# quentinll/pertrenderer

Hardware: AMD Instinct MI355X
Metric: rendered frames/sec + ms/backward, 256² img, 50 faces/px, 8 samples (higher is better)
Workload: dtype f32; 1 GPU; cfg2 pose-opt step: sphere_642 (1280 faces), 256x256, faces_per_pixel=50, Sr=Sa=8 Gaussian, sigma=1e-3 gamma=1e-2, blur=ln(1e4-1)*sigma, fwd + L2 loss (native) + bwd + Adam step on the pose (lr 5e-2); image_size=256, faces_per_pixel=50, nb_samples=8, rast_samples=8, batch=1, execution=graph, parallelism=single GPU

## Files before the change

### pertrenderer_amd/csrc/pr_rast.hip

```cpp
#include <cstdlib>
#include <type_traits>

#include <hip/hip_fp16.h>

#include "pr_common.h"

namespace pr {
namespace {

constexpr float kEps = 1e-8f;
constexpr int kTile = 4;

struct V2 {
  float x, y;
};

template <bool FAST = false>
PR_DEV float dv(float a, float b) {
  if constexpr (FAST) return a * __builtin_amdgcn_rcpf(b);
  else return a / b;
}

PR_DEV float edge_fn(V2 p, V2 a, V2 b) { return (p.x - a.x) * (b.y - a.y) - (p.y - a.y) * (b.x - a.x); }

// ... 396 lines not shown
        const int je = j >> 6;
#pragma unroll
        for (int e = 0; e < E; ++e) {
          const int pe = e ^ je;
          if (pe > e) {
            const bool up = ((e * 64 + lane) & k) == 0;
            const float a = key[e], b = key[pe];
            if ((a > b) == up) {
              key[e] = b; key[pe] = a;
              const int t = val[e]; val[e] = val[pe]; val[pe] = t;
            }
          }
        }
      } else {
#pragma unroll
        for (int e = 0; e < E; ++e) {
          const float ok = __shfl_xor(key[e], j);
          const int ov = __shfl_xor(val[e], j);
          const int i = e * 64 + lane;
          const bool up = (i & k) == 0, lower = (lane & j) == 0;
          const bool take = lower == up ? (ok < key[e]) : (ok > key[e]);
          if (take) { key[e] = ok; val[e] = ov; }
        }
      }
    }
  }
}

template <int E>
PR_DEV void wave_sort_lds(float* lkey, int* lidx, int lane) {
  float kk[E];
  int vv[E];
#pragma unroll
  for (int e = 0; e < E; ++e) { kk[e] = lkey[e * 64 + lane]; vv[e] = lidx[e * 64 + lane]; }
  wave_bitonic_sort<E>(kk, vv, lane);
#pragma unroll
  for (int e = 0; e < E; ++e) { lkey[e * 64 + lane] = kk[e]; lidx[e * 64 + lane] = vv[e]; }
}

PR_DEV bool ekey_less(float2 x, float2 y) { return key_less(x.x, __float_as_int(x.y), y.x, __float_as_int(y.y)); }

template <int SL>
PR_HD size_t rast_fwd_wave_bytes(int K) {
  using C = RastCfg<SL>;
  const size_t b = C::CH * sizeof(FaceRec) + (size_t)K * (64 / SL + rast_qpad<SL>()) * 8 + 64 * 4 + C::CH * 12;
  return (b + 15) / 16 * 16;
}

template <int SL>
size_t rast_fwd_lds_sl(int K, int NW) {
  return NW * rast_fwd_wave_bytes<SL>(K) + (size_t)RastCfg<SL>::CAP * 12 + 16;
}

size_t rast_fwd_lds(int K, int SL, int NW = 1) {
  return SL == 8 ? rast_fwd_lds_sl<8>(K, 1)
                 : SL == 4 ? rast_fwd_lds_sl<4>(K, NW) : (SL == 2 ? rast_fwd_lds_sl<2>(K, 1) : rast_fwd_lds_sl<1>(K, 1));
}

template <int SL>
PR_DEV int from_slice(int v, int s) {
  if constexpr (SL == 1) {
    return v;
  } else if constexpr (SL == 2) {
    switch (s) {
      case 0: return __builtin_amdgcn_update_dpp(0, v, 0xA0, 0xf, 0xf, false);
      default: return __builtin_amdgcn_update_dpp(0, v, 0xF5, 0xf, 0xf, false);
    }
  } else if constexpr (SL == 8) {
    return __shfl(v, (int)(__lane_id() & ~7u) | s);
  } else {
    switch (s) {
      case 0: return __builtin_amdgcn_update_dpp(0, v, 0x00, 0xf, 0xf, false);
      case 1: return __builtin_amdgcn_update_dpp(0, v, 0x55, 0xf, 0xf, false);
      case 2: return __builtin_amdgcn_update_dpp(0, v, 0xAA, 0xf, 0xf, false);
      default: return __builtin_amdgcn_update_dpp(0, v, 0xFF, 0xf, 0xf, false);
    }
  }
}

template <int SL>
PR_DEV int quad_rot(int v, int r) {
  if constexpr (SL == 2) {
    return __builtin_amdgcn_update_dpp(0, v, 0xB1, 0xf, 0xf, false);
  } else if constexpr (SL == 8) {
    const unsigned l = __lane_id();
    return __shfl(v, (int)((l & ~7u) | ((l + (unsigned)r) & 7u)));
  } else {
    switch (r) {
      case 1: return __builtin_amdgcn_update_dpp(0, v, 0x39, 0xf, 0xf, false);
      case 2: return __builtin_amdgcn_update_dpp(0, v, 0x4E, 0xf, 0xf, false);
      default: return __builtin_amdgcn_update_dpp(0, v, 0x93, 0xf, 0xf, false);
    }
  }
}

PR_DEV int64_t uniform64(int64_t v) {
  return (int64_t)(((uint64_t)(uint32_t)__builtin_amdgcn_readfirstlane((int)(v >> 32)) << 32) |
                   (uint32_t)__builtin_amdgcn_readfirstlane((int)v));
}

PR_DEV void ring_tile(int b, int m, int& tx, int& ty) {
  int r = (int)(__builtin_sqrtf((float)b) * 0.5f);
  while (4 * (r + 1) * (r + 1) <= b) ++r;
  while (4 * r * r > b) --r;
  const int k = b - 4 * r * r, s = 2 * r + 2, c0 = m / 2 - r - 1;
  if (k < s) { tx = c0 + k; ty = c0; }
  else if (k < 2 * s - 2) { tx = c0 + s - 1; ty = c0 + 1 + (k - s); }
  else if (k < 3 * s - 2) { tx = c0 + s - 1 - (k - (2 * s - 2)); ty = c0 + s - 1; }
  else { tx = c0; ty = c0 + s - 2 - (k - (3 * s - 2)); }
}

#ifndef PR_RAST_WPE
#define PR_RAST_WPE 1
#endif
#ifndef PR_RAST_DUO_WPE
#define PR_RAST_DUO_WPE 1
#endif
template <int SL, bool PERSP, bool CLIP, bool FRAG, int NW>
__global__ void __launch_bounds__(64 * NW, NW == 2 ? PR_RAST_DUO_WPE : PR_RAST_WPE)
    rast_fwd_kernel(PRRastArgs a, const FaceRec* __restrict__ faces, const uint2* __restrict__ fbox,
                    int chunk_cull, int ring, BinGrid bins) {
  constexpr int TW = SL >= 4 ? 4 : 8, TH = 64 / SL / TW, TP = TW * TH;
  constexpr int kCap = RastCfg<SL>::CAP, kGroup = RastCfg<SL>::G, CH = RastCfg<SL>::CH;
  constexpr int QS = TP + rast_qpad<SL>();
  constexpr int NT = 64 * NW;
  extern __shared__ float smem[];
  const int K = a.K;
  const int tid = threadIdx.x, lane = tid & 63, wv = NW == 2 ? tid >> 6 : 0;
  const int pix = lane / SL, slice = lane % SL;
  const size_t wbytes = rast_fwd_wave_bytes<SL>(K);
  char* wbase = reinterpret_cast<char*>(smem) + wv * wbytes;
  FaceRec* lrec = reinterpret_cast<FaceRec*>(wbase);
  float2* q = reinterpret_cast<float2*>(lrec + CH);
  int* qsz = reinterpret_cast<int*>(q + (size_t)K * QS);
  int* lcf = qsz + 64;
  float* lcs = reinterpret_cast<float*>(lcf + CH);
  float* lmg = lcs + CH;
  int* lfid = reinterpret_cast<int*>(reinterpret_cast<char*>(smem) + NW * wbytes);
  float* lkey = reinterpret_cast<float*>(lfid + kCap);
  float* lsuf = lkey;
  int* lidx = reinterpret_cast<int*>(lkey + kCap);
  int64_t* lctl = reinterpret_cast<int64_t*>(lidx + kCap);
  int* lscr = reinterpret_cast<int*>(lctl);
  const int n = blockIdx.z;
  const int H = a.H, W = a.W;
  int tile_x = blockIdx.x, tile_y = blockIdx.y;
  if (ring & 1) {
    const int b = blockIdx.y * gridDim.x + blockIdx.x;
    if (gridDim.y == gridDim.x) {
      ring_tile(b, gridDim.x, tile_x, tile_y);
    } else {
      ring_tile(b >> 1, gridDim.x, tile_x, tile_y);
      tile_y = 2 * tile_y + (b & 1);
    }
  }
  const int row0 = tile_y * TH, col0 = tile_x * TW;
  const int row = row0 + pix / TW, col = col0 + pix % TW;
  const bool inimg = row < H && col < W;
  const V2 p{ndc(W - 1 - min(col, W - 1), W, H), ndc(H - 1 - min(row, H - 1), H, W)};
  const int c1 = min(col0 + TW - 1, W - 1), r1 = min(row0 + TH - 1, H - 1);
  const float txmax = ndc(W - 1 - col0, W, H), txmin = ndc(W - 1 - c1, W, H);
  const float tymax = ndc(H - 1 - row0, H, W), tymin = ndc(H - 1 - r1, H, W);
  const float tcx = 0.5f * (txmin + txmax), tcy = 0.5f * (tymin + tymax);
  const float ptile = fmaxf(fmaxf(fabsf(txmin), fabsf(txmax)), fmaxf(fabsf(tymin), fabsf(tymax)));
  const int64_t fb = a.mesh_first_face[n];
  const int* ids = nullptr;
  int64_t fe = a.mesh_num_faces[n];
  if (bins.count) {
    const int b = (n * bins.ny + row0 / bins.bs) * bins.nx + col0 / bins.bs;
    const int c = bins.count[b];
    if (c <= bins.cap) { ids = bins.list + (int64_t)b * bins.cap; fe = c; }
  }
  constexpr bool clip = CLIP;
  const float blur = a.blur_radius_dev ? *a.blur_radius_dev : a.blur_radius, sqrt_blur = sqrtf(blur);
  int qs = 0;
  float qlast_z = __builtin_inff();
  int qlast_f = 0x7fffffff;
  int64_t base = 0;
#ifdef PR_RAST_PROFILE
  long long stamp[6] = {0, 0, 0, 0, 0, 0}, t_ = __builtin_amdgcn_s_memtime();
  const long long rt0 = __builtin_amdgcn_s_memrealtime();
  int nlist = 0, n_app = 0, n_ins = 0, w_ins = 0;
#endif
  while (base < fe) {
    int nl = 0;
    if (__builtin_amdgcn_readfirstlane(ids == nullptr && wv == 0)) {
      const int64_t ufb = uniform64(fb), ufe = uniform64(fe);
      const int f_lo = (int)ufb, f_hi = (int)(ufb + ufe);
      const int cN = (int)((ufb + ufe - 1) / kChunk) + 1;
      int64_t ub = uniform64(base);
      int un = 0;
      while (ub < ufe && un <= kCap - 64) {
        const int c0 = (int)((ufb + ub) / kChunk);
        bool ck = c0 + lane < cN;
        if (ck && chunk_cull) {
          const float4 cb = unpack_box(fbox[(c0 + lane) * kChunk]);
          ck = !(cb.x > txmax || cb.y < txmin || cb.z > tymax || cb.w < tymin);
        }
        uint64_t live = __ballot(ck);
        const int64_t wend = (int64_t)(c0 + 64 < cN ? c0 + 64 : cN) * kChunk - ufb;
        int64_t next = wend;
        while (live != 0 && un <= kCap - 64) {
          uint2 pb[kChunkU];
          const uint64_t live0 = live;
          const int nlive = __popcll(live);
          const int np = nlive < kChunkU ? nlive : kChunkU;
          int g = -1;
#pragma unroll
          for (int u = 0; u < kChunkU; ++u) {
            pb[u] = make_uint2(0u, 0u);
            if (u < np) {
              const int f0 = (c0 + __builtin_ctzll(live)) * kChunk, f = f0 + lane;
              live &= live - 1;
              pb[u] = fbox[f >= f_lo && f < f_hi ? f : f_lo];
              if (lane == u) g = f0;
            }
          }
          float4 ex = make_float4(0.f, 0.f, 0.f, 0.f);
          if (g >= f_lo && g < f_hi) ex = exact_box(faces + g);
          uint64_t lv = live0;
          int stop = -1;
#pragma unroll
          for (int u = 0; u < kChunkU; ++u) {
            if (u < np && stop < 0) {
              const uint64_t lv0 = lv;
              const int f = (c0 + __builtin_ctzll(lv)) * kChunk + lane;
              lv &= lv - 1;
              float4 bb = unpack_box(pb[u]);
              const float e0 = __shfl(ex.x, u), e1 = __shfl(ex.y, u), e2 = __shfl(ex.z, u), e3 = __shfl(ex.w, u);
              if (lane == 0) bb = make_float4(e0, e1, e2, e3);
              const bool keep = f >= f_lo && f < f_hi && !(bb.x > txmax || bb.y < txmin || bb.z > tymax || bb.w < tymin);
              const uint64_t bal = __ballot(keep);
              const int cnt = __popcll(bal);
              if (un + cnt > kCap) {
                stop = u;
                live = lv0;
              } else {
                *(keep ? lfid + un + __popcll(bal & ((1ull << lane) - 1ull)) : lscr) = f;
                un += cnt;
              }
            }
          }
          next = live != 0 ? (int64_t)(c0 + __builtin_ctzll(live)) * kChunk - ufb : wend;
          if (stop >= 0) live = 0;
        }
        next = next > ub ? next : ub;
        ub = next < ufe ? next : ufe;
      }
      base = ub;
      nl = un;
    }
    while (wv == 0 && base < fe && nl <= kCap - 64) {
      uint2 pb[kCullU];
      int fi[kCullU];
#pragma unroll
      for (int u = 0; u < kCullU; ++u) {
        const int64_t i = base + u * 64 + lane;
        const int64_t ic = i < fe ? i : fe - 1;
        fi[u] = ids ? ids[ic] : (int)(fb + ic);
      }
#pragma unroll
      for (int u = 0; u < kCullU; ++u) pb[u] = fbox[fi[u]];
      int64_t next = base + 64 * kCullU;
      bool stop = false;
#pragma unroll
      for (int u = 0; u < kCullU; ++u) {
        const int64_t i = base + u * 64 + lane;
        float4 bb = unpack_box(pb[u]);
        if ((fi[u] & (kChunk - 1)) == 0) bb = exact_box(faces + fi[u]);
        const bool keep = i < fe && !(bb.x > txmax || bb.y < txmin || bb.z > tymax || bb.w < tymin);
        const uint64_t bal = __ballot(keep);
        const int cnt = __popcll(bal);
        if (!stop && nl + cnt > kCap) { stop = true; next = base + u * 64; }
        if (!stop) {
          if (keep) lfid[nl + __popcll(bal & ((1ull << lane) - 1ull))] = fi[u];
          nl += cnt;
        }
      }
      base = next < fe ? next : fe;
    }
    if constexpr (NW > 1) {
      if (tid == 0) { lctl[0] = base; lctl[1] = nl; }
      __syncthreads();
      base = lctl[0];
      nl = (int)lctl[1];
    }
    __syncthreads();
    PR_STAMP(0);
#ifdef PR_RAST_PROFILE
    nlist += nl;
#endif
    if (nl == 0) continue;
    if (ring & 2) {
      const int t = ring >> 8;
      if (nl >= t + 32) __builtin_amdgcn_s_setprio(3);
      else if (nl >= t + 16) __builtin_amdgcn_s_setprio(2);
      else if (nl >= t) __builtin_amdgcn_s_setprio(1);
    }
    bool done = !inimg;
    int n2 = 64;
    while (n2 < nl) n2 <<= 1;
    for (int i = tid; i < n2; i += NT) {
      float key = __builtin_inff();
      if (i < nl) {
        const FaceRec& r = faces[lfid[i]];
        const float4 ra = r.a, rb = r.b, re = r.e, rf = r.f;
        const float z2 = r.c.x, area = r.d.y;
        const float e0 = (tcx - ra.w) * re.w - (tcy - rb.x) * re.z;
        const float e1 = (tcx - rb.z) * rf.y - (tcy - rb.w) * rf.x;
        const float e2 = (tcx - ra.x) * re.y - (tcy - ra.y) * re.x;
        const float ia = 1.f / area;
        const float zc = (e0 * ia) * ra.z + (e1 * ia) * rb.y + (e2 * ia) * z2;
        const float zmx = fmaxf(ra.z, fmaxf(rb.y, z2));
        key = fminf(fmaxf(zc, rf.w), zmx);
        if (key != key) key = rf.w;
        key = fminf(key, 3.0e38f);
        if (key != key) key = 0.f;
      }
      lkey[i] = key;
      lidx[i] = i < nl ? i : 0x7fffffff;
    }
    __syncthreads();
    PR_STAMP(1);
    if (wv == 0) {
      if (n2 == 64) wave_sort_lds<1>(lkey, lidx, lane);
      else if (kCap >= 128 && n2 == 128) wave_sort_lds<2>(lkey, lidx, lane);
      else if (kCap >= 256 && n2 == 256) wave_sort_lds<4>(lkey, lidx, lane);
      else if constexpr (kCap >= 512) wave_sort_lds<8>(lkey, lidx, lane);
    }
    __syncthreads();
    PR_STAMP(2);
    {
      const int per = (nl + 63) / 64;
      const int i0 = lane * per, i1 = wv == 0 ? min(nl, i0 + per) : i0;
      float zl[8];
#pragma unroll
      for (int u = 0; u < 8; ++u) zl[u] = i0 + u < i1 ? faces[lfid[lidx[i0 + u]]].f.w : __builtin_inff();
      float m = __builtin_inff();
#pragma unroll
      for (int u = 0; u < 8; ++u) m = fminf(m, zl[u]);
      float ex = m;
#pragma unroll
      for (int o = 1; o < 64; o <<= 1) {
        const float t = __shfl_down(ex, o);
        if (lane + o < 64) ex = fminf(ex, t);
      }
      float run = __shfl_down(ex, 1);
      if (lane == 63) run = __builtin_inff();
      __syncthreads();
#pragma unroll
      for (int u = 7; u >= 0; --u) {
        run = fminf(run, zl[u]);
        if (i0 + u < i1) lsuf[i0 + u] = run;
      }
    }
    __syncthreads();
    PR_STAMP(3);
    float4 nra, nrb, nrc, nrd, nre, nrf;
    int nfid = 0;
    float nsuf = 0.f;
    if (lane < CH) {
      const int sp = min(wv * CH + lane, nl - 1);
      nfid = lfid[lidx[sp]];
      nsuf = lsuf[sp];
      const FaceRec* fp = faces + nfid;
      nra = fp->a; nrb = fp->b; nrc = fp->c; nrd = fp->d; nre = fp->e; nrf = fp->f;
    }
    for (int c0 = wv * CH; c0 < nl && __ballot(!done) != 0; c0 += NW * CH) {
      const int cnt = min(CH, nl - c0);
      __builtin_amdgcn_wave_barrier();
      if (lane < cnt) {
        FaceRec& d = lrec[lane];
        d.a = nra; d.b = nrb; d.c = nrc; d.d = nrd; d.e = nre; d.f = nrf;
        lcf[lane] = nfid;
        lcs[lane] = nsuf;
        if constexpr (!PERSP) lmg[lane] = dist_margin(nra, nrb, ptile, sqrt_blur, blur);
      }
      __builtin_amdgcn_fence(__ATOMIC_RELEASE, "wavefront");
      __builtin_amdgcn_wave_barrier();
      if (c0 + NW * CH < nl && lane < CH) {
        const int sp = c0 + NW * CH + min(lane, nl - c0 - NW * CH - 1);
        nfid = lfid[lidx[sp]];
        nsuf = lsuf[sp];
        const FaceRec* fp = faces + nfid;
        nra = fp->a; nrb = fp->b; nrc = fp->c; nrd = fp->d; nre = fp->e; nrf = fp->f;
      }
      const int steps = (cnt + SL - 1) / SL;
      for (int t = 0; t < steps; t += kGroup) {
        bool cand[kGroup], ok[kGroup];
        float pzv[kGroup];
        int idx[kGroup];
        FaceRec rr[kGroup];
        bool any = false;
#pragma unroll
        for (int j = 0; j < kGroup; ++j) {
          idx[j] = (t + j) * SL + slice;
          ok[j] = idx[j] < cnt;
          rr[j] = lrec[min(idx[j], cnt - 1)];
        }
        bool maybe[kGroup];
        float dfast[kGroup], mg[kGroup];
#pragma unroll
        for (int j = 0; j < kGroup; ++j) {
          dfast[j] = 0.f;
          mg[j] = PERSP ? 0.f : lmg[min(idx[j], cnt - 1)];
          if constexpr (PERSP) maybe[j] = ok[j] && in_bbox(rr[j], p);
          else maybe[j] = ok[j] && face_maybe(rr[j], p, blur, mg[j], dfast[j]);
          any |= __ballot(maybe[j]) != 0;
        }
// ... 108 lines not shown
            const bool enter = mine && !done && cand[j] && (qs < K || key_less(pz, fid, qlast_z, qlast_f));
            if (__ballot(enter) == 0) continue;
            {
              if (enter) {
                if (qs == 0 || key_less(qlast_z, qlast_f, pz, fid)) {
                  q[qs * QS + pix] = make_float2(pz, __int_as_float(fid));
                  ++qs;
                  qlast_z = pz;
                  qlast_f = fid;
#ifdef PR_RAST_PROFILE
                  ++n_app;
#endif
                } else {
#ifdef PR_RAST_PROFILE
                  ++n_ins;
#endif
                  int pos = qs < K ? qs : K - 1;
                  if (qs < K) ++qs;
                  while (pos > 0) {
                    float2 e[4];
#pragma unroll
                    for (int i = 0; i < 4; ++i) e[i] = q[max(pos - 1 - i, 0) * QS + pix];
                    int sh = 0;
#pragma unroll
                    for (int i = 0; i < 4; ++i) {
                      if (sh == i && pos - 1 - i >= 0 && key_less(pz, fid, e[i].x, __float_as_int(e[i].y))) {
                        q[(pos - i) * QS + pix] = e[i];
                        sh = i + 1;
                      }
                    }
                    pos -= sh;
                    if (sh < 4) break;
                  }
                  q[pos * QS + pix] = make_float2(pz, __int_as_float(fid));
                  const float2 last = q[(qs - 1) * QS + pix];
                  qlast_z = last.x;
                  qlast_f = __float_as_int(last.y);
                }
              }
            }
            if constexpr (SL > 1) {
              qs = from_slice<SL>(qs, sl);
              qlast_z = __int_as_float(from_slice<SL>(__float_as_int(qlast_z), sl));
              qlast_f = from_slice<SL>(qlast_f, sl);
            }
          }
        }
#ifdef PR_RAST_PROFILE
        w_ins += __ballot(n_ins != ins_before) != 0;
#endif
        if (__ballot(!done) == 0) break;
      }
    }
    __syncthreads();
    PR_STAMP(4);
  }
  if (slice == 0) qsz[pix] = inimg ? qs : 0;
  if constexpr (NW == 1) {
    if (slice == 0 && inimg && a.pix_count) a.pix_count[((int64_t)n * H + row) * W + col] = qs;
  }
  __syncthreads();
  const float2* qa = reinterpret_cast<const float2*>(reinterpret_cast<const char*>(lrec) - wv * wbytes + CH * sizeof(FaceRec));
  const float2* qb = reinterpret_cast<const float2*>(reinterpret_cast<const char*>(qa) + wbytes);
  const int* qsa = reinterpret_cast<const int*>(qa + (size_t)K * QS);
  const int* qsb = reinterpret_cast<const int*>(qb + (size_t)K * QS);
  if constexpr (NW == 2) {
    if (wv == 0 && slice == 0 && inimg && a.pix_count)
      a.pix_count[((int64_t)n * H + row) * W + col] = min(K, qsa[pix] + qsb[pix]);
  }
  auto msize = [&](int t) { return NW == 2 ? min(K, qsa[t] + qsb[t]) : qsz[t]; };
  auto kth = [&](int t, int k) -> float2 {
    if constexpr (NW == 1) {
      return q[k * QS + t];
    } else {
      const int na = qsa[t], nb = qsb[t];
      int lo = max(0, k - nb), hi = min(k, na);
      while (lo < hi) {
        const int mid = (lo + hi) >> 1;
        if (ekey_less(qa[mid * QS + t], qb[(k - 1 - mid) * QS + t])) lo = mid + 1;
        else hi = mid;
      }
      const int j = k - lo;
      if (lo >= na) return qb[j * QS + t];
      if (j >= nb) return qa[lo * QS + t];
      const float2 x = qa[lo * QS + t], y = qb[j * QS + t];
      return ekey_less(x, y) ? x : y;
    }
  };
  {
    const int ncols = min(TW, W - col0), nrows = min(TH, H - row0);
    const int per_row = ncols * K, total = nrows * per_row;
    const float inv_row = 1.f / (float)per_row, inv_k = 1.f / (float)K;
#ifndef PR_RAST_OUTU
#define PR_RAST_OUTU 4
#endif
    constexpr int U = PR_RAST_OUTU;
    constexpr bool kCompact = FRAG && TP <= 16 && PR_RAST_FRAGC;
    const bool valid_only = kCompact && a.pix_count && (a.flags & PR_RAST_VALID_ONLY);
    for (int base = 0; base < (valid_only ? 0 : total); base += NT * U) {
      float2 e[U];
      int sz[U], kk[U], cc[U], rr[U];
      int64_t o[U];
#pragma unroll
      for (int u = 0; u < U; ++u) {
        const int i = min(base + u * NT + tid, total - 1);
        int rem;
        rr[u] = divmod_small(i, per_row, inv_row, rem);
        cc[u] = divmod_small(rem, K, inv_k, kk[u]);
        const int tl = rr[u] * TW + cc[u];
        o[u] = (((int64_t)n * H + row0 + rr[u]) * W + col0) * K + rem;
        sz[u] = msize(tl);
        if constexpr (NW == 1) e[u] = q[kk[u] * QS + tl];
        else e[u] = kk[u] < sz[u] ? kth(tl, kk[u]) : make_float2(0.f, 0.f);
      }
// ... 32 lines not shown
      const int mysz = lane < TP ? msize(lane) : 0;
      int incl = mysz;
#pragma unroll
      for (int o = 1; o < TP; o <<= 1) {
        const int t = __shfl_up(incl, o);
        if (lane >= o) incl += t;
      }
      const int excl = incl - mysz;
      int ex[TP];
#pragma unroll
      for (int t = 0; t < TP; ++t) ex[t] = __builtin_amdgcn_readlane(excl, t);
      const int nvalid = __builtin_amdgcn_readlane(incl, TP - 1);
      for (int vb = 0; vb < nvalid; vb += NT * U) {
        float2 e[U];
        int tl[U], kk[U];
#pragma unroll
        for (int u = 0; u < U; ++u) {
          const int v = min(vb + u * NT + tid, nvalid - 1);
          int t = 0, e0 = 0;
#pragma unroll
          for (int s = 1; s < TP; ++s) {
            const bool ge = v >= ex[s];
            t = ge ? s : t;
            e0 = ge ? ex[s] : e0;
          }
          tl[u] = t;
          kk[u] = v - e0;
          e[u] = kth(t, kk[u]);
        }
#pragma unroll
        for (int u = 0; u < U; ++u) {
          if (vb + u * NT + tid >= nvalid) break;
          const int fid = __float_as_int(e[u].y);
          const int rr = tl[u] / TW, cc = tl[u] % TW;
          const int64_t o = (((int64_t)n * H + row0 + rr) * W + col0 + cc) * K + kk[u];
          const V2 pp{ndc(W - 1 - (col0 + cc), W, H), ndc(H - 1 - (row0 + rr), H, W)};
          const FaceRec r = faces[fid];
          float bc[3], pz, d;
          bool inside;
          face_eval<PERSP, CLIP>(r, pp, bc, pz, inside, d);
          if (valid_only) {
            a.pix_to_face[o] = (int64_t)fid;
            a.zbuf[o] = e[u].x;
          }
          a.dists[o] = inside ? -d : d;
          a.bary[o * 3 + 0] = bc[0];
          a.bary[o * 3 + 1] = bc[1];
          a.bary[o * 3 + 2] = bc[2];
        }
      }
    }
  }
#ifdef PR_RAST_PROFILE
  __syncthreads();
  PR_STAMP(5);
  int n_app_tot = n_app, n_ins_tot = n_ins;
  for (int o = 32; o > 0; o >>= 1) { n_app_tot += __shfl_xor(n_app_tot, o); n_ins_tot += __shfl_xor(n_ins_tot, o); }
  if (tid == 0) {
    unsigned hw, xcc;
    asm volatile("s_getreg_b32 %0, hwreg(HW_REG_HW_ID)" : "=s"(hw));
    asm volatile("s_getreg_b32 %0, hwreg(HW_REG_XCC_ID)" : "=s"(xcc));
    const unsigned t = (blockIdx.z * gridDim.y + blockIdx.y) * gridDim.x + blockIdx.x;
    if (t < kProfTiles) {
      long long* rec = g_rast_prof + (size_t)t * 16;
      rec[0] = tile_x; rec[1] = tile_y; rec[2] = blockIdx.z; rec[3] = nlist;
      rec[4] = rt0; rec[5] = (long long)__builtin_amdgcn_s_memrealtime();
      rec[6] = (long long)hw | ((long long)(xcc & 0xf) << 32);
      for (int i = 0; i < 6; ++i) rec[7 + i] = stamp[i];
      rec[13] = SL;
      rec[14] = n_app_tot;
      rec[15] = ((long long)n_ins_tot << 32) | (unsigned)w_ins;
    }
  }
#endif
}

template <int SL, bool PERSP, bool CLIP>
void launch_rast_fwd_sl(const PRRastArgs& a, const FaceRec* fr, const uint2* fb, int cc, bool frag, size_t lds,
                        const BinGrid& bins, hipStream_t st, int nw) {
  constexpr int TW = SL >= 4 ? 4 : 8, TH = 64 / SL / TW;
  dim3 grid((a.W + TW - 1) / TW, (a.H + TH - 1) / TH, a.N);
  static const bool ring_env = (getenv("PR_RAST_ORDER") ? atoi(getenv("PR_RAST_ORDER")) : 3) & 1;
  static const bool prio_env = getenv("PR_RAST_PRIO") ? atoi(getenv("PR_RAST_PRIO")) != 0 : true;
  static const int prio_t = getenv("PR_RAST_PRIO_T") ? atoi(getenv("PR_RAST_PRIO_T")) & 255 : 40;
  const bool sq = grid.x % 2 == 0 && (grid.y == grid.x || grid.y == 2 * grid.x);
  const int ring = (ring_env && sq ? 1 : 0) | (prio_env ? 2 : 0) | (prio_t << 8);
  ktimer_mark(0, "rast_fwd_kernel", st);
  if constexpr (SL == 4) {
    if (nw == 2) {
      if (frag) rast_fwd_kernel<SL, PERSP, CLIP, true, 2><<<grid, 128, lds, st>>>(a, fr, fb, cc, ring, bins);
      else rast_fwd_kernel<SL, PERSP, CLIP, false, 2><<<grid, 128, lds, st>>>(a, fr, fb, cc, ring, bins);
      ktimer_mark(1, "rast_fwd_kernel", st);
      return;
    }
  }
  if (frag) rast_fwd_kernel<SL, PERSP, CLIP, true, 1><<<grid, 64, lds, st>>>(a, fr, fb, cc, ring, bins);
  else rast_fwd_kernel<SL, PERSP, CLIP, false, 1><<<grid, 64, lds, st>>>(a, fr, fb, cc, ring, bins);
  ktimer_mark(1, "rast_fwd_kernel", st);
}

template <bool PERSP, bool CLIP>
void launch_rast_fwd_pc(const PRRastArgs& a, const FaceRec* fr, const uint2* fb, int cc, int sl, bool frag,
                        size_t lds, const BinGrid& bins, hipStream_t st, int nw) {
  if (sl == 8) launch_rast_fwd_sl<8, PERSP, CLIP>(a, fr, fb, cc, frag, lds, bins, st, 1);
  else if (sl == 4) launch_rast_fwd_sl<4, PERSP, CLIP>(a, fr, fb, cc, frag, lds, bins, st, nw);
  else if (sl == 2) launch_rast_fwd_sl<2, PERSP, CLIP>(a, fr, fb, cc, frag, lds, bins, st, 1);
  else launch_rast_fwd_sl<1, PERSP, CLIP>(a, fr, fb, cc, frag, lds, bins, st, 1);
}

void launch_rast_fwd(const PRRastArgs& a, const FaceRec* fr, const uint2* fb, int cc, int sl, bool frag,
                     size_t lds, const BinGrid& bins, hipStream_t st, int nw) {
  const bool persp = a.perspective_correct != 0, clip = a.clip_barycentric_coords != 0;
  if (persp && clip) launch_rast_fwd_pc<true, true>(a, fr, fb, cc, sl, frag, lds, bins, st, nw);
  else if (persp) launch_rast_fwd_pc<true, false>(a, fr, fb, cc, sl, frag, lds, bins, st, nw);
  else if (clip) launch_rast_fwd_pc<false, true>(a, fr, fb, cc, sl, frag, lds, bins, st, nw);
  else launch_rast_fwd_pc<false, false>(a, fr, fb, cc, sl, frag, lds, bins, st, nw);
}

template <bool WIDE>
__global__ void __launch_bounds__(kThreads) rast_frag_kernel(PRRastArgs a, int64_t total) {
  using idx_t = typename std::conditional<WIDE, int64_t, uint32_t>::type;
  const bool persp = a.perspective_correct != 0, clip = a.clip_barycentric_coords != 0;
  for (int64_t oo = (int64_t)blockIdx.x * kThreads + threadIdx.x; oo < total; oo += (int64_t)gridDim.x * kThreads) {
    const idx_t o = (idx_t)oo;
    const int64_t fid = a.pix_to_face[o];
    float bc[3] = {-1.f, -1.f, -1.f}, dist = -1.f;
    if (fid >= 0) {
      const idx_t pix = o / (idx_t)a.K;
      const int col = (int)(pix % (idx_t)a.W), row = (int)((pix / (idx_t)a.W) % (idx_t)a.H);
      const V2 pp{ndc(a.W - 1 - col, a.W, a.H), ndc(a.H - 1 - row, a.H, a.W)};
      const float* v = a.face_verts + fid * 9;
      const V2 v0{v[0], v[1]}, v1{v[3], v[4]}, v2{v[6], v[7]};
      float b0[3], b[3];
      bary_fwd(pp, v0, v1, v2, b0);
      if (persp) persp_fwd(b0, v[2], v[5], v[8], b); else { b[0] = b0[0]; b[1] = b0[1]; b[2] = b0[2]; }
      if (clip) clip_fwd(b, bc); else { bc[0] = b[0]; bc[1] = b[1]; bc[2] = b[2]; }
      const bool inside = b[0] > 0.f && b[1] > 0.f && b[2] > 0.f;
      const float d = tri_dist2(pp, v0, v1, v2);
      dist = inside ? -d : d;
    }
    a.dists[o] = dist;
    a.bary[o * 3 + 0] = bc[0];
    a.bary[o * 3 + 1] = bc[1];
    a.bary[o * 3 + 2] = bc[2];
  }
}

PR_DEV void seg_dist2_bwd(V2 p, V2 a, V2 b, float g, V2& ga, V2& gb) {
  const float bax = b.x - a.x, bay = b.y - a.y;
  const float l2 = bax * bax + bay * bay;
  float t;
  if (l2 <= kEps) t = 1.f;
  else {
    t = dv<true>(bax * (p.x - a.x) + bay * (p.y - a.y), l2);
    t = t < 0.f ? 0.f : (t > 1.f ? 1.f : t);
  }
  const float qx = (1.f - t) * a.x + t * b.x, qy = (1.f - t) * a.y + t * b.y;
  const float dx = qx - p.x, dy = qy - p.y;
  ga.x = g * (1.f - t) * 2.f * dx; ga.y = g * (1.f - t) * 2.f * dy;
  gb.x = g * t * 2.f * dx;         gb.y = g * t * 2.f * dy;
}

PR_DEV void tri_dist2_bwd(V2 p, V2 v0, V2 v1, V2 v2, float g, V2 gv[3]) {
  const float e01 = seg_dist2(p, v0, v1), e02 = seg_dist2(p, v0, v2), e12 = seg_dist2(p, v1, v2);
  gv[0] = V2{0.f, 0.f}; gv[1] = V2{0.f, 0.f}; gv[2] = V2{0.f, 0.f};
  if (e01 <= e02 && e01 <= e12) seg_dist2_bwd(p, v0, v1, g, gv[0], gv[1]);
  else if (e02 <= e01 && e02 <= e12) seg_dist2_bwd(p, v0, v2, g, gv[0], gv[2]);
  else seg_dist2_bwd(p, v1, v2, g, gv[1], gv[2]);
}
// ... 709 lines not shown
  if (g.bs == 0) return 0;
  const size_t nb = (size_t)a.N * g.ny * g.nx;
  return nb * sizeof(int) * (1 + (size_t)g.cap);
}

extern "C" size_t pr_rast_fwd_workspace_size(const PRRastArgs* a) {
  if (!a) return 0;
  return (size_t)(a->F > 0 ? a->F : 1) * (sizeof(FaceRec) + sizeof(uint2)) + bin_bytes(*a);
}

static int bins_begin(const PRRastArgs& a, BinGrid& g, hipStream_t st) {
  g = bin_grid(a, a.workspace);
  if (!g.count) return PR_OK;
  if (hipMemsetAsync(g.count, 0, (size_t)a.N * g.ny * g.nx * sizeof(int), st) != hipSuccess)
    return set_error(PR_ERR_HIP, "rast_fwd: bin counter memset failed");
  return PR_OK;
}

static int rast_fwd_prepared(const PRRastArgs& a, const FaceRec* fr, const uint2* fbox, const BinGrid& bins,
                             hipStream_t st);

extern "C" int pr_rast_fwd(const PRRastArgs* args, void* stream) {
  if (!args) return set_error(PR_ERR_ARG, "rast_fwd: null args");
  const PRRastArgs& a = *args;
  if (int e = rast_check(a)) return e;
  if (!a.pix_to_face || !a.zbuf || !a.bary || !a.dists) return set_error(PR_ERR_ARG, "rast_fwd: output missing");
  if (!a.workspace || a.workspace_bytes < pr_rast_fwd_workspace_size(args))
    return set_error(PR_ERR_WORKSPACE, "rast_fwd: workspace too small");
  hipStream_t st = reinterpret_cast<hipStream_t>(stream);
  FaceRec* fr = reinterpret_cast<FaceRec*>(a.workspace);
  uint2* fbox = reinterpret_cast<uint2*>(fr + (a.F > 0 ? a.F : 1));
  BinGrid bins;
  if (int e = bins_begin(a, bins, st)) return e;
  if (a.F > 0) {
    const int nb = (int)std::min<int64_t>((a.F + kThreads - 1) / kThreads, 1024);
    face_prep_kernel<<<nb, kThreads, 0, st>>>(a.face_verts, a.F, a.blur_radius, a.blur_radius_dev, a.cull_backfaces, fr,
                                              fbox, bins, a.mesh_first_face, a.N);
    if (int e = check_launch("rast_face_prep")) return e;
  }
  return rast_fwd_prepared(a, fr, fbox, bins, st);
}

static int rast_fwd_prepared(const PRRastArgs& a, const FaceRec* fr, const uint2* fbox, const BinGrid& bins,
                             hipStream_t st) {
  int sl = (int64_t)a.K * 16 * 8 > 16 * 1024 ? 8 : 4;
  if (const char* e = getenv("PR_RAST_SLICES")) {
    const int v = atoi(e);
    if (v == 1 || v == 2 || v == 4 || v == 8) sl = v;
  }
  bool frag = true;
  if (const char* e = getenv("PR_RAST_FRAG")) frag = atoi(e) != 0;
  const char* duo = getenv("PR_RAST_DUO");
  const int nw = sl == 4 && duo && duo[0] == '1' ? 2 : 1;
  size_t lds = rast_fwd_lds(a.K, sl, nw);
  if (const char* e = getenv("PR_RAST_LDS_MIN")) lds = std::max(lds, (size_t)atol(e));
  if (lds > 160 * 1024) return set_error(PR_ERR_ARG, "rast_fwd: faces_per_pixel too large for the LDS queue (max 300)");
  const char* cc = getenv("PR_RAST_CHUNK_CULL");
  const int chunk_cull = !(cc && cc[0] == '0');
  launch_rast_fwd(a, fr, fbox, chunk_cull, sl, frag, lds, bins, st, nw);
  if (int e = check_launch("rast_fwd")) return e;
  if (frag) return PR_OK;
  const int64_t total = (int64_t)a.N * a.H * a.W * a.K;
  const int nb = (int)std::min<int64_t>((total + kThreads - 1) / kThreads, 1 << 20);
  if (total * 3 < (int64_t(1) << 32)) rast_frag_kernel<false><<<nb, kThreads, 0, st>>>(a, total);
  else rast_frag_kernel<true><<<nb, kThreads, 0, st>>>(a, total);
  return check_launch("rast_frag");
}

extern "C" size_t pr_rast_bwd_workspace_size(const PRRastArgs* a) {
  if (!a || !(a->flags & PR_DETERMINISTIC)) return 0;
  return detsum_workspace(std::min<int64_t>((int64_t)a->N * a->H * a->W * a->K, det_batch()), a->F, 9);
}

static int rast_bwd_deterministic(const PRRastArgs& a, hipStream_t st) {
  const int64_t total = (int64_t)a.N * a.H * a.W * a.K, batch = det_batch();
  if (a.F == 0) return PR_OK;
  for (int64_t s0 = 0; s0 < total; s0 += batch) {
    const int64_t n = std::min(batch, total - s0);
    DetSum d;
    if (int e = detsum_layout(a.workspace, a.workspace_bytes, n, a.F, 9, d)) return e;
    const int nb = (int)std::min<int64_t>((n + kThreads - 1) / kThreads, 16384);
    rast_bwd_keys_kernel<<<nb, kThreads, 0, st>>>(a, d.keys, s0, n);
    if (int e = check_launch("rast_bwd_keys")) return e;
    if (int e = detsum_sort(d, st)) return e;
    rast_bwd_sorted_grad_kernel<<<nb, kThreads, 0, st>>>(a, d.keys_sorted, d.idx_sorted, d.vals_sorted, s0, n);
    if (int e = check_launch("rast_bwd_sorted_grad")) return e;
    if (int e = detsum_reduce_chain(d, a.grad_face_verts, s0 == 0, st)) return e;
  }
  return PR_OK;
}

extern "C" int pr_rast_bwd(const PRRastArgs* args, void* stream) {
  if (!args) return set_error(PR_ERR_ARG, "rast_bwd: null args");
  const PRRastArgs& a = *args;
  if (int e = rast_check(a)) return e;
  if (!a.pix_to_face || !a.grad_face_verts) return set_error(PR_ERR_ARG, "rast_bwd: buffer missing");
  hipStream_t st = reinterpret_cast<hipStream_t>(stream);
  if (a.flags & PR_DETERMINISTIC) return rast_bwd_deterministic(a, st);
  if (a.F > 0 && !(a.flags & PR_GRAD_PREZEROED)) {
    if (hipMemsetAsync(a.grad_face_verts, 0, (size_t)a.F * 9 * sizeof(float), st) != hipSuccess)
      return set_error(PR_ERR_HIP, "rast_bwd: memset failed");
  }
  const char* er = getenv("PR_RAST_BWD_ROWS");
  const int64_t npix = (int64_t)a.N * a.H * a.W;
  const int rows = er && (atoi(er) == 1 || atoi(er) == 2 || atoi(er) == 4 || atoi(er) == 8) ? atoi(er)
                                                                                            : (npix >= (1 << 18) ? 4 : 2);
  dim3 grid((a.W + kBwdTile - 1) / kBwdTile, (a.H + rows - 1) / rows, a.N);
  static const int order = (getenv("PR_RAST_ORDER") ? atoi(getenv("PR_RAST_ORDER")) : 3) >> 1 & 1;
  static const bool exact = !getenv("PR_RAST_BWD_EXACT") || atoi(getenv("PR_RAST_BWD_EXACT")) != 0;
#define PR_RAST_BWD_LAUNCH(R)                                               \
  do {                                                                      \
    if (exact) rast_bwd_kernel<R, true><<<grid, kBwdThreads, 0, st>>>(a, order);  \
// ... 98 lines not shown
```

Before: 4040 frames/s (fwd+bwd).

## Add 4-wave quad-tile rasterizer sharing face culling and presorted depth list

Adds a QUAD variant of the forward rasterizer: 256-thread blocks, each covering a 2x2 group of 4x4-pixel wave tiles. The four waves cull the mesh's chunks against the group bounding box together, building one shared face list in LDS. By default each block then ranks that list by depth once, so each wave only filters it against its own tile and skips the per-tile depth sort. Waves sync with wave barriers instead of block barriers. It is enabled by default for K<=53 when no binning is used. The cost is a block-wide barrier, more LDS per block, and a depth order taken at the group centre instead of each tile's centre.

```diff
diff --git a/pertrenderer_amd/csrc/pr_rast.hip b/pertrenderer_amd/csrc/pr_rast.hip
--- a/pertrenderer_amd/csrc/pr_rast.hip
+++ b/pertrenderer_amd/csrc/pr_rast.hip
@@ -472,7 +472,15 @@
   return NW * rast_fwd_wave_bytes<SL>(K) + (size_t)RastCfg<SL>::CAP * 12 + 16;
 }
 
-size_t rast_fwd_lds(int K, int SL, int NW = 1) {
+constexpr int kQuadSeg = 128, kQuadList = 256;
+constexpr int kQuadMaxK = 53;
+PR_HD size_t rast_fwd_quad_wave_bytes(int K) { return rast_fwd_wave_bytes<4>(K) + (size_t)RastCfg<4>::CAP * 12 + 16; }
+PR_HD size_t rast_fwd_quad_lds(int K) {
+  return 4 * rast_fwd_quad_wave_bytes(K) + (size_t)(4 * kQuadSeg + 1) * 16 + (size_t)(4 * kQuadSeg + 4 + 4 + kQuadList) * 4;
+}
+
+size_t rast_fwd_lds(int K, int SL, int NW = 1, bool quad = false) {
+  if (quad) return rast_fwd_quad_lds(K);
   return SL == 8 ? rast_fwd_lds_sl<8>(K, 1)
                  : SL == 4 ? rast_fwd_lds_sl<4>(K, NW) : (SL == 2 ? rast_fwd_lds_sl<2>(K, 1) : rast_fwd_lds_sl<1>(K, 1));
 }
@@ -536,27 +544,57 @@
 #ifndef PR_RAST_DUO_WPE
 #define PR_RAST_DUO_WPE 1
 #endif
-template <int SL, bool PERSP, bool CLIP, bool FRAG, int NW>
-__global__ void __launch_bounds__(64 * NW, NW == 2 ? PR_RAST_DUO_WPE : PR_RAST_WPE)
+PR_DEV float depth_key(const FaceRec& r, float cx, float cy) {
+  const float4 ra = r.a, rb = r.b, re = r.e, rf = r.f;
+  const float z2 = r.c.x, area = r.d.y;
+  const float e0 = (cx - ra.w) * re.w - (cy - rb.x) * re.z;
+  const float e1 = (cx - rb.z) * rf.y - (cy - rb.w) * rf.x;
+  const float e2 = (cx - ra.x) * re.y - (cy - ra.y) * re.x;
+  const float ia = 1.f / area;
+  const float zc = (e0 * ia) * ra.z + (e1 * ia) * rb.y + (e2 * ia) * z2;
+  const float zmx = fmaxf(ra.z, fmaxf(rb.y, z2));
+  float key = fminf(fmaxf(zc, rf.w), zmx);
+  if (key != key) key = rf.w;
+  key = fminf(key, 3.0e38f);
+  if (key != key) key = 0.f;
+  return key;
+}
+
+template <bool QUAD>
+PR_DEV void tile_sync() {
+  if constexpr (QUAD) {
+    __builtin_amdgcn_fence(__ATOMIC_RELEASE, "wavefront");
+    __builtin_amdgcn_wave_barrier();
+    __builtin_amdgcn_fence(__ATOMIC_ACQUIRE, "wavefront");
+  } else {
+    __syncthreads();
+  }
+}
+
+template <int SL, bool PERSP, bool CLIP, bool FRAG, int NW, bool QUAD = false>
+__global__ void __launch_bounds__(QUAD ? 256 : 64 * NW, NW == 2 ? PR_RAST_DUO_WPE : PR_RAST_WPE)
     rast_fwd_kernel(PRRastArgs a, const FaceRec* __restrict__ faces, const uint2* __restrict__ fbox,
                     int chunk_cull, int ring, BinGrid bins) {
+  static_assert(!QUAD || (SL == 4 && NW == 1), "the quad instance is the one-wave 4-slice tile path");
   constexpr int TW = SL >= 4 ? 4 : 8, TH = 64 / SL / TW, TP = TW * TH;
   constexpr int kCap = RastCfg<SL>::CAP, kGroup = RastCfg<SL>::G, CH = RastCfg<SL>::CH;
   constexpr int QS = TP + rast_qpad<SL>();
   constexpr int NT = 64 * NW;
   extern __shared__ float smem[];
   const int K = a.K;
-  const int tid = threadIdx.x, lane = tid & 63, wv = NW == 2 ? tid >> 6 : 0;
+  const int tid = QUAD ? threadIdx.x & 63 : threadIdx.x, lane = tid & 63, wv = NW == 2 ? tid >> 6 : 0;
+  const int qw = QUAD ? __builtin_amdgcn_readfirstlane(threadIdx.x >> 6) : 0;
   const int pix = lane / SL, slice = lane % SL;
   const size_t wbytes = rast_fwd_wave_bytes<SL>(K);
-  char* wbase = reinterpret_cast<char*>(smem) + wv * wbytes;
+  const size_t wstride = QUAD ? wbytes + (size_t)kCap * 12 + 16 : wbytes;
+  char* wbase = reinterpret_cast<char*>(smem) + (QUAD ? qw : wv) * wstride;
   FaceRec* lrec = reinterpret_cast<FaceRec*>(wbase);
   float2* q = reinterpret_cast<float2*>(lrec + CH);
   int* qsz = reinterpret_cast<int*>(q + (size_t)K * QS);
   int* lcf = qsz + 64;
   float* lcs = reinterpret_cast<float*>(lcf + CH);
   float* lmg = lcs + CH;
-  int* lfid = reinterpret_cast<int*>(reinterpret_cast<char*>(smem) + NW * wbytes);
+  int* lfid = reinterpret_cast<int*>(QUAD ? wbase + wbytes : reinterpret_cast<char*>(smem) + NW * wbytes);
   float* lkey = reinterpret_cast<float*>(lfid + kCap);
   float* lsuf = lkey;
   int* lidx = reinterpret_cast<int*>(lkey + kCap);
@@ -565,7 +603,9 @@
   const int n = blockIdx.z;
   const int H = a.H, W = a.W;
   int tile_x = blockIdx.x, tile_y = blockIdx.y;
-  if (ring & 1) {
+  if constexpr (QUAD) {
+    if (ring & 1) ring_tile(blockIdx.y * gridDim.x + blockIdx.x, gridDim.x, tile_x, tile_y);
+  } else if (ring & 1) {
     const int b = blockIdx.y * gridDim.x + blockIdx.x;
     if (gridDim.y == gridDim.x) {
       ring_tile(b, gridDim.x, tile_x, tile_y);
@@ -573,6 +613,15 @@
       ring_tile(b >> 1, gridDim.x, tile_x, tile_y);
       tile_y = 2 * tile_y + (b & 1);
     }
+  }
+  float gxmin = 0.f, gxmax = 0.f, gymin = 0.f, gymax = 0.f;
+  if constexpr (QUAD) {
+    const int gc0 = tile_x * 2 * TW, gr0 = tile_y * 2 * TH;
+    const int gc1 = min(gc0 + 2 * TW - 1, a.W - 1), gr1 = min(gr0 + 2 * TH - 1, a.H - 1);
+    gxmax = ndc(a.W - 1 - gc0, a.W, a.H); gxmin = ndc(a.W - 1 - gc1, a.W, a.H);
+    gymax = ndc(a.H - 1 - gr0, a.H, a.W); gymin = ndc(a.H - 1 - gr1, a.H, a.W);
+    tile_x = 2 * tile_x + (qw & 1);
+    tile_y = 2 * tile_y + (qw >> 1);
   }
   const int row0 = tile_y * TH, col0 = tile_x * TW;
   const int row = row0 + pix / TW, col = col0 + pix % TW;
@@ -586,7 +635,7 @@
   const int64_t fb = a.mesh_first_face[n];
   const int* ids = nullptr;
   int64_t fe = a.mesh_num_faces[n];
-  if (bins.count) {
+  if (!QUAD && bins.count) {
     const int b = (n * bins.ny + row0 / bins.bs) * bins.nx + col0 / bins.bs;
     const int c = bins.count[b];
     if (c <= bins.cap) { ids = bins.list + (int64_t)b * bins.cap; fe = c; }
@@ -602,9 +651,138 @@
   const long long rt0 = __builtin_amdgcn_s_memrealtime();
   int nlist = 0, n_app = 0, n_ins = 0, w_ins = 0;
 #endif
-  while (base < fe) {
+  bool use_list = false;
+  int gtot = 0, gp1 = 0, gp2 = 0, gp3 = 0;
+  float4* gbox = nullptr;
+  int* gfid = nullptr;
+  const float* gzl = nullptr;
+  if constexpr (QUAD) {
+    gbox = reinterpret_cast<float4*>(reinterpret_cast<char*>(smem) + 4 * wstride);
+    gfid = reinterpret_cast<int*>(gbox + 4 * kQuadSeg + 1);
+    int* gcnt = gfid + 4 * kQuadSeg + 4;
+    const int64_t ufb = uniform64(fb), ufe = uniform64(fe);
+    const int f_lo = (int)ufb, f_hi = (int)(ufb + ufe);
+    const int c0 = (int)(ufb / kChunk), cN = ufe > 0 ? (int)((ufb + ufe - 1) / kChunk) + 1 : c0;
+    const bool one_window = cN - c0 <= 64;
+    int sn = 0;
+    bool over = false;
+    if (one_window && ufe > 0) {
+      bool ck = c0 + lane < cN;
+      if (ck && chunk_cull) {
+        const float4 cb = unpack_box(fbox[(c0 + lane) * kChunk]);
+        ck = !(cb.x > gxmax || cb.y < gxmin || cb.z > gymax || cb.w < gymin);
+      }
+      const uint64_t all = __ballot(ck);
+      const int rank = __popcll(all & ((1ull << lane) - 1ull));
+      uint64_t live = __ballot(ck && (rank & 3) == qw);
+      const int np = __popcll(live);
+      static_assert(kChunkU >= 16, "a wave's share of a 64-chunk window is one group of passes");
+      uint2 pb[16];
+      const uint64_t live0 = live;
+      int g = -1;
+#pragma unroll
+      for (int u = 0; u < 16; ++u) {
+        pb[u] = make_uint2(0u, 0u);
+        if (u < np) {
+          const int f0 = (c0 + __builtin_ctzll(live)) * kChunk, f = f0 + lane;
+          live &= live - 1;
+          pb[u] = fbox[f >= f_lo && f < f_hi ? f : f_lo];
+          if (lane == u) g = f0;
+        }
+      }
+      float4 ex = make_float4(0.f, 0.f, 0.f, 0.f);
+      if (g >= f_lo && g < f_hi) ex = exact_box(faces + g);
+      uint64_t lv = live0;
+      float4* sbox = gbox + qw * kQuadSeg;
+      int* sfid = gfid + qw * kQuadSeg;
+#pragma unroll
+      for (int u = 0; u < 16; ++u) {
+        if (u < np && !over) {
+          const int f = (c0 + __builtin_ctzll(lv)) * kChunk + lane;
+          lv &= lv - 1;
+          float4 bb = unpack_box(pb[u]);
+          const float e0 = __shfl(ex.x, u), e1 = __shfl(ex.y, u), e2 = __shfl(ex.z, u), e3 = __shfl(ex.w, u);
+          if (lane == 0) bb = make_float4(e0, e1, e2, e3);
+          const bool keep = f >= f_lo && f < f_hi && !(bb.x > gxmax || bb.y < gxmin || bb.z > gymax || bb.w < gymin);
+          const uint64_t bal = __ballot(keep);
+          const int cnt = __popcll(bal);
+          if (sn + cnt > kQuadSeg) {
+            over = true;
+          } else {
+            const int at = keep ? sn + __popcll(bal & ((1ull << lane) - 1ull)) : -1;
+            *(at >= 0 ? sbox + at : gbox + 4 * kQuadSeg) = bb;
+            *(at >= 0 ? sfid + at : gfid + 4 * kQuadSeg) = f;
+            sn += cnt;
+          }
+        }
+      }
+    }
+    if (lane == 0) gcnt[qw] = over ? kQuadList + 1 : sn;
+    __syncthreads();
+    const int n0 = gcnt[0], n1 = gcnt[1], n2 = gcnt[2], n3 = gcnt[3];
+    gp1 = n0; gp2 = n0 + n1; gp3 = n0 + n1 + n2; gtot = gp3 + n3;
+    use_list = __builtin_amdgcn_readfirstlane(one_window && gtot <= kQuadList);
+    if (use_list && (ring & 4)) {
+      unsigned* gkey = reinterpret_cast<unsigned*>(reinterpret_cast<char*>(smem) + wbytes);
+      float* gz = reinterpret_cast<float*>(gcnt + 4);
+      static_assert(kQuadList == 256 && kQuadList * 4 <= RastCfg<4>::CAP * 12, "one entry per thread; keys fit a wave's list");
+      const int t = threadIdx.x;
+      float4 bb = make_float4(0.f, 0.f, 0.f, 0.f);
+      int f = 0;
+      float key = __builtin_inff(), zmin = 0.f;
+      if (t < gtot) {
+        const int sg = (t >= gp1 ? 1 : 0) + (t >= gp2 ? 1 : 0) + (t >= gp3 ? 1 : 0);
+        const int e = sg * kQuadSeg + t - (sg == 0 ? 0 : (sg == 1 ? gp1 : (sg == 2 ? gp2 : gp3)));
+        bb = gbox[e];
+        f = gfid[e];
+        const FaceRec& r = faces[f];
+        key = depth_key(r, 0.5f * (gxmin + gxmax), 0.5f * (gymin + gymax));
+        zmin = r.f.w;
+      }
+      unsigned kb = __float_as_uint(key);
+      kb = (kb & 0x80000000u) ? ~kb : kb | 0x80000000u;
+      const unsigned kw = t < gtot ? (kb & ~255u) | (unsigned)t : 0xffffffffu;
+      gkey[t] = kw;
+      __syncthreads();
+      int rank = 0;
+      for (int j0 = 0; j0 < gtot; j0 += 16) {
+        uint4 k4[4];
+#pragma unroll
+        for (int u = 0; u < 4; ++u) k4[u] = *reinterpret_cast<const uint4*>(gkey + j0 + 4 * u);
+#pragma unroll
+        for (int u = 0; u < 4; ++u)
+          rank += (k4[u].x < kw ? 1 : 0) + (k4[u].y < kw ? 1 : 0) + (k4[u].z < kw ? 1 : 0) + (k4[u].w < kw ? 1 : 0);
+      }
+      if (t < gtot) { gbox[rank] = bb; gfid[rank] = f; gz[rank] = zmin; }
+      __syncthreads();
+      gp1 = gp2 = gp3 = 0x7fffffff;
+      gzl = gz;
+    }
+    if (col0 >= W || row0 >= H) return;
+  }
+  const int64_t rend = use_list ? (int64_t)gtot : fe;
+  while (base < rend) {
     int nl = 0;
-    if (__builtin_amdgcn_readfirstlane(ids == nullptr && wv == 0)) {
+    if (QUAD && use_list) {
+      int un = 0, gp = __builtin_amdgcn_readfirstlane((int)base);
+      while (gp < gtot && un <= kCap - 64) {
+        const int j = gp + lane;
+        const bool v = j < gtot;
+        const int s = (j >= gp1 ? 1 : 0) + (j >= gp2 ? 1 : 0) + (j >= gp3 ? 1 : 0);
+        const int e = v ? s * kQuadSeg + j - (s == 0 ? 0 : (s == 1 ? gp1 : (s == 2 ? gp2 : gp3))) : 0;
+        const float4 bb = gbox[e];
+        const int f = gfid[e];
+        const bool keep = v && !(bb.x > txmax || bb.y < txmin || bb.z > tymax || bb.w < tymin);
+        const uint64_t bal = __ballot(keep);
+        const int at = un + __popcll(bal & ((1ull << lane) - 1ull));
+        *(keep ? lfid + at : lscr) = f;
+        if (gzl && keep) { lkey[at] = gzl[e]; lidx[at] = at; }
+        un += __popcll(bal);
+        gp += 64;
+      }
+      base = gp < gtot ? gp : gtot;
+      nl = un;
+    } else if (__builtin_amdgcn_readfirstlane(ids == nullptr && wv == 0)) {
       const int64_t ufb = uniform64(fb), ufe = uniform64(fe);
       const int f_lo = (int)ufb, f_hi = (int)(ufb + ufe);
       const int cN = (int)((ufb + ufe - 1) / kChunk) + 1;
@@ -670,7 +848,7 @@
       base = ub;
       nl = un;
     }
-    while (wv == 0 && base < fe && nl <= kCap - 64) {
+    while (!(QUAD && use_list) && wv == 0 && base < fe && nl <= kCap - 64) {
       uint2 pb[kCullU];
       int fi[kCullU];
 #pragma unroll
@@ -705,7 +883,7 @@
       base = lctl[0];
       nl = (int)lctl[1];
     }
-    __syncthreads();
+    tile_sync<QUAD>();
     PR_STAMP(0);
 #ifdef PR_RAST_PROFILE
     nlist += nl;
@@ -718,44 +896,32 @@
       else if (nl >= t) __builtin_amdgcn_s_setprio(1);
     }
     bool done = !inimg;
+    const bool presorted = QUAD && use_list && (ring & 4);
     int n2 = 64;
     while (n2 < nl) n2 <<= 1;
-    for (int i = tid; i < n2; i += NT) {
+    for (int i = tid; i < (presorted ? 0 : n2); i += NT) {
       float key = __builtin_inff();
-      if (i < nl) {
-        const FaceRec& r = faces[lfid[i]];
-        const float4 ra = r.a, rb = r.b, re = r.e, rf = r.f;
-        const float z2 = r.c.x, area = r.d.y;
-        const float e0 = (tcx - ra.w) * re.w - (tcy - rb.x) * re.z;
-        const float e1 = (tcx - rb.z) * rf.y - (tcy - rb.w) * rf.x;
-        const float e2 = (tcx - ra.x) * re.y - (tcy - ra.y) * re.x;
-        const float ia = 1.f / area;
-        const float zc = (e0 * ia) * ra.z + (e1 * ia) * rb.y + (e2 * ia) * z2;
-        const float zmx = fmaxf(ra.z, fmaxf(rb.y, z2));
-        key = fminf(fmaxf(zc, rf.w), zmx);
-        if (key != key) key = rf.w;
-        key = fminf(key, 3.0e38f);
-        if (key != key) key = 0.f;
-      }
+      if (i < nl) key = depth_key(faces[lfid[i]], tcx, tcy);
       lkey[i] = key;
       lidx[i] = i < nl ? i : 0x7fffffff;
     }
-    __syncthreads();
+    tile_sync<QUAD>();
     PR_STAMP(1);
-    if (wv == 0) {
+    if (wv == 0 && !presorted) {
       if (n2 == 64) wave_sort_lds<1>(lkey, lidx, lane);
       else if (kCap >= 128 && n2 == 128) wave_sort_lds<2>(lkey, lidx, lane);
       else if (kCap >= 256 && n2 == 256) wave_sort_lds<4>(lkey, lidx, lane);
       else if constexpr (kCap >= 512) wave_sort_lds<8>(lkey, lidx, lane);
     }
-    __syncthreads();
+    tile_sync<QUAD>();
     PR_STAMP(2);
     {
       const int per = (nl + 63) / 64;
       const int i0 = lane * per, i1 = wv == 0 ? min(nl, i0 + per) : i0;
       float zl[8];
 #pragma unroll
-      for (int u = 0; u < 8; ++u) zl[u] = i0 + u < i1 ? faces[lfid[lidx[i0 + u]]].f.w : __builtin_inff();
+      for (int u = 0; u < 8; ++u)
+        zl[u] = i0 + u < i1 ? (presorted ? lkey[i0 + u] : faces[lfid[lidx[i0 + u]]].f.w) : __builtin_inff();
       float m = __builtin_inff();
 #pragma unroll
       for (int u = 0; u < 8; ++u) m = fminf(m, zl[u]);
@@ -767,14 +933,14 @@
       }
       float run = __shfl_down(ex, 1);
       if (lane == 63) run = __builtin_inff();
-      __syncthreads();
+      tile_sync<QUAD>();
 #pragma unroll
       for (int u = 7; u >= 0; --u) {
         run = fminf(run, zl[u]);
         if (i0 + u < i1) lsuf[i0 + u] = run;
       }
     }
-    __syncthreads();
+    tile_sync<QUAD>();
     PR_STAMP(3);
     float4 nra, nrb, nrc, nrd, nre, nrf;
     int nfid = 0;
@@ -989,14 +1155,14 @@
         if (__ballot(!done) == 0) break;
       }
     }
-    __syncthreads();
+    tile_sync<QUAD>();
     PR_STAMP(4);
   }
   if (slice == 0) qsz[pix] = inimg ? qs : 0;
   if constexpr (NW == 1) {
     if (slice == 0 && inimg && a.pix_count) a.pix_count[((int64_t)n * H + row) * W + col] = qs;
   }
-  __syncthreads();
+  tile_sync<QUAD>();
   const float2* qa = reinterpret_cast<const float2*>(reinterpret_cast<const char*>(lrec) - wv * wbytes + CH * sizeof(FaceRec));
   const float2* qb = reinterpret_cast<const float2*>(reinterpret_cast<const char*>(qa) + wbytes);
   const int* qsa = reinterpret_cast<const int*>(qa + (size_t)K * QS);
@@ -1135,7 +1301,7 @@
     }
   }
 #ifdef PR_RAST_PROFILE
-  __syncthreads();
+  tile_sync<QUAD>();
   PR_STAMP(5);
   int n_app_tot = n_app, n_ins_tot = n_ins;
   for (int o = 32; o > 0; o >>= 1) { n_app_tot += __shfl_xor(n_app_tot, o); n_ins_tot += __shfl_xor(n_ins_tot, o); }
@@ -1143,7 +1309,7 @@
     unsigned hw, xcc;
     asm volatile("s_getreg_b32 %0, hwreg(HW_REG_HW_ID)" : "=s"(hw));
     asm volatile("s_getreg_b32 %0, hwreg(HW_REG_XCC_ID)" : "=s"(xcc));
-    const unsigned t = (blockIdx.z * gridDim.y + blockIdx.y) * gridDim.x + blockIdx.x;
+    const unsigned t = ((blockIdx.z * gridDim.y + blockIdx.y) * gridDim.x + blockIdx.x) * (QUAD ? 4 : 1) + qw;
     if (t < kProfTiles) {
       long long* rec = g_rast_prof + (size_t)t * 16;
       rec[0] = tile_x; rec[1] = tile_y; rec[2] = blockIdx.z; rec[3] = nlist;
@@ -1160,16 +1326,23 @@
 
 template <int SL, bool PERSP, bool CLIP>
 void launch_rast_fwd_sl(const PRRastArgs& a, const FaceRec* fr, const uint2* fb, int cc, bool frag, size_t lds,
-                        const BinGrid& bins, hipStream_t st, int nw) {
+                        const BinGrid& bins, hipStream_t st, int nw, int quad) {
   constexpr int TW = SL >= 4 ? 4 : 8, TH = 64 / SL / TW;
   dim3 grid((a.W + TW - 1) / TW, (a.H + TH - 1) / TH, a.N);
+  if (quad) grid = dim3((a.W + 2 * TW - 1) / (2 * TW), (a.H + 2 * TH - 1) / (2 * TH), a.N);
   static const bool ring_env = (getenv("PR_RAST_ORDER") ? atoi(getenv("PR_RAST_ORDER")) : 3) & 1;
   static const bool prio_env = getenv("PR_RAST_PRIO") ? atoi(getenv("PR_RAST_PRIO")) != 0 : true;
   static const int prio_t = getenv("PR_RAST_PRIO_T") ? atoi(getenv("PR_RAST_PRIO_T")) & 255 : 40;
-  const bool sq = grid.x % 2 == 0 && (grid.y == grid.x || grid.y == 2 * grid.x);
-  const int ring = (ring_env && sq ? 1 : 0) | (prio_env ? 2 : 0) | (prio_t << 8);
+  const bool sq = grid.x % 2 == 0 && (grid.y == grid.x || (!quad && grid.y == 2 * grid.x));
+  const int ring = (ring_env && sq ? 1 : 0) | (prio_env ? 2 : 0) | (quad == 2 ? 4 : 0) | (prio_t << 8);
   ktimer_mark(0, "rast_fwd_kernel", st);
   if constexpr (SL == 4) {
+    if (quad) {
+      if (frag) rast_fwd_kernel<SL, PERSP, CLIP, true, 1, true><<<grid, 256, lds, st>>>(a, fr, fb, cc, ring, bins);
+      else rast_fwd_kernel<SL, PERSP, CLIP, false, 1, true><<<grid, 256, lds, st>>>(a, fr, fb, cc, ring, bins);
+      ktimer_mark(1, "rast_fwd_kernel", st);
+      return;
+    }
     if (nw == 2) {
       if (frag) rast_fwd_kernel<SL, PERSP, CLIP, true, 2><<<grid, 128, lds, st>>>(a, fr, fb, cc, ring, bins);
       else rast_fwd_kernel<SL, PERSP, CLIP, false, 2><<<grid, 128, lds, st>>>(a, fr, fb, cc, ring, bins);
@@ -1184,20 +1357,20 @@
 
 template <bool PERSP, bool CLIP>
 void launch_rast_fwd_pc(const PRRastArgs& a, const FaceRec* fr, const uint2* fb, int cc, int sl, bool frag,
-                        size_t lds, const BinGrid& bins, hipStream_t st, int nw) {
-  if (sl == 8) launch_rast_fwd_sl<8, PERSP, CLIP>(a, fr, fb, cc, frag, lds, bins, st, 1);
-  else if (sl == 4) launch_rast_fwd_sl<4, PERSP, CLIP>(a, fr, fb, cc, frag, lds, bins, st, nw);
-  else if (sl == 2) launch_rast_fwd_sl<2, PERSP, CLIP>(a, fr, fb, cc, frag, lds, bins, st, 1);
-  else launch_rast_fwd_sl<1, PERSP, CLIP>(a, fr, fb, cc, frag, lds, bins, st, 1);
+                        size_t lds, const BinGrid& bins, hipStream_t st, int nw, int quad) {
+  if (sl == 8) launch_rast_fwd_sl<8, PERSP, CLIP>(a, fr, fb, cc, frag, lds, bins, st, 1, 0);
+  else if (sl == 4) launch_rast_fwd_sl<4, PERSP, CLIP>(a, fr, fb, cc, frag, lds, bins, st, nw, quad);
+  else if (sl == 2) launch_rast_fwd_sl<2, PERSP, CLIP>(a, fr, fb, cc, frag, lds, bins, st, 1, 0);
+  else launch_rast_fwd_sl<1, PERSP, CLIP>(a, fr, fb, cc, frag, lds, bins, st, 1, 0);
 }
 
 void launch_rast_fwd(const PRRastArgs& a, const FaceRec* fr, const uint2* fb, int cc, int sl, bool frag,
-                     size_t lds, const BinGrid& bins, hipStream_t st, int nw) {
+                     size_t lds, const BinGrid& bins, hipStream_t st, int nw, int quad) {
   const bool persp = a.perspective_correct != 0, clip = a.clip_barycentric_coords != 0;
-  if (persp && clip) launch_rast_fwd_pc<true, true>(a, fr, fb, cc, sl, frag, lds, bins, st, nw);
-  else if (persp) launch_rast_fwd_pc<true, false>(a, fr, fb, cc, sl, frag, lds, bins, st, nw);
-  else if (clip) launch_rast_fwd_pc<false, true>(a, fr, fb, cc, sl, frag, lds, bins, st, nw);
-  else launch_rast_fwd_pc<false, false>(a, fr, fb, cc, sl, frag, lds, bins, st, nw);
+  if (persp && clip) launch_rast_fwd_pc<true, true>(a, fr, fb, cc, sl, frag, lds, bins, st, nw, quad);
+  else if (persp) launch_rast_fwd_pc<true, false>(a, fr, fb, cc, sl, frag, lds, bins, st, nw, quad);
+  else if (clip) launch_rast_fwd_pc<false, true>(a, fr, fb, cc, sl, frag, lds, bins, st, nw, quad);
+  else launch_rast_fwd_pc<false, false>(a, fr, fb, cc, sl, frag, lds, bins, st, nw, quad);
 }
 
 template <bool WIDE>
@@ -2013,12 +2186,18 @@
   if (const char* e = getenv("PR_RAST_FRAG")) frag = atoi(e) != 0;
   const char* duo = getenv("PR_RAST_DUO");
   const int nw = sl == 4 && duo && duo[0] == '1' ? 2 : 1;
-  size_t lds = rast_fwd_lds(a.K, sl, nw);
+  const char* qe = getenv("PR_RAST_QUAD");
+  const bool quad_ok = sl == 4 && nw == 1 && !bins.count;
+  const bool quad = quad_ok && rast_fwd_quad_lds(a.K) <= 64 * 1024 &&
+                    (qe && (qe[0] == '0' || qe[0] == '1') ? qe[0] == '1' : a.K <= kQuadMaxK);
+  const char* qs = getenv("PR_RAST_QUAD_SORT");
+  const int quad_mode = !quad ? 0 : (qs && qs[0] == 't' ? 1 : 2);
+  size_t lds = rast_fwd_lds(a.K, sl, nw, quad);
   if (const char* e = getenv("PR_RAST_LDS_MIN")) lds = std::max(lds, (size_t)atol(e));
   if (lds > 160 * 1024) return set_error(PR_ERR_ARG, "rast_fwd: faces_per_pixel too large for the LDS queue (max 300)");
   const char* cc = getenv("PR_RAST_CHUNK_CULL");
   const int chunk_cull = !(cc && cc[0] == '0');
-  launch_rast_fwd(a, fr, fbox, chunk_cull, sl, frag, lds, bins, st, nw);
+  launch_rast_fwd(a, fr, fbox, chunk_cull, sl, frag, lds, bins, st, nw, quad_mode);
   if (int e = check_launch("rast_fwd")) return e;
   if (frag) return PR_OK;
   const int64_t total = (int64_t)a.N * a.H * a.W * a.K;
```

After: 4073 frames/s (fwd+bwd), median of 6. No clear change (+0.8%).
